# blasif/cocons

Hardware: NVIDIA B200
Metric: neg2loglik evals/sec (assembly+Cholesky) at n=50k (higher is better)
Workload: dtype f64

## Files before the change

### cocons_b200/csrc/capi.cu

```cuda
#include <algorithm>
#include <atomic>
#include <iterator>
#include <cmath>
#include <cstdarg>
#include <cstdio>
#include <cstring>
#include <mutex>
#include <vector>

#include "../../include/cocons_b200.h"
#include "common.cuh"

namespace cocons {

static thread_local char g_err[512] = "";
void set_error(const char* fmt, ...) {
  va_list ap;
  va_start(ap, fmt);
  vsnprintf(g_err, sizeof(g_err), fmt, ap);
  va_end(ap);
}

static std::atomic<long long> g_launches{0};
void note_launch(int count) { g_launches += count; }
// ... 1534 lines not shown
    cudaSetDevice(c->device);
    morton_order(n, locs, c->perm.data());
    c->hX.assign(X, X + (size_t)n * p);
    c->rank_x = -1;
    cudaFree(c->dInv), cudaFree(c->dTapCol), cudaFree(c->dTapRow), cudaFree(c->dTap);
    c->dInv = c->dTapCol = c->dTapRow = nullptr, c->dTap = nullptr, c->tap_nnz = 0;
    std::vector<int> orig((size_t)c->n_pad);
    for (int64_t s = 0; s < c->n_pad; ++s) orig[(size_t)s] = (s < n) ? (int)c->perm[(size_t)s] : (int)s;
    COCONS_CUDA_TRY(cudaMemcpy(c->dOrig, orig.data(), sizeof(int) * c->n_pad, cudaMemcpyHostToDevice));
    if ((rc = upload_sorted(c, X, p, c->dX)) || (rc = upload_sorted(c, locs, 2, c->dLocs)) ||
        (rc = upload_sorted(c, z, r, c->dZ)))
      return rc;
  }
  if (kind == COCONS_PROFILE) {
    if (!xb || q <= 0) {
      set_error("neg2loglik_dense: COCONS_PROFILE needs x_betas");
      return COCONS_ERR_ARG;
    }
    if ((rc = cocons_ctx_set_xbetas(g_ws, q, xb))) return rc;
  }
  return cocons_n2ll(g_ws, kind, theta6, limits, mean_p, logdet, quad, logdet_w, rank_x);
}


__global__ void fill_kernel(double* p, int64_t count, double scale) {
  const int64_t i = (int64_t)blockIdx.x * blockDim.x + threadIdx.x;
  if (i < count) p[i] = scale * (double)(((uint64_t)i * 2654435761ull) % 1024ull) / 1024.0;
}

int cocons_bench_syrk(int device, int64_t n, int64_t k, int reps, double* ms_per_rep) {
  int rc = check_device(device);
  if (rc) return rc;
  if (n % kTile || k % 16 || !ms_per_rep || reps <= 0) {
    set_error("bench_syrk: n must be a multiple of 128 and k of 16");
    return COCONS_ERR_ARG;
  }
  double *dC = nullptr, *dP = nullptr;
  COCONS_CUDA_TRY(cudaMalloc(&dC, sizeof(double) * n * n));
  if (cudaMalloc(&dP, sizeof(double) * n * k) != cudaSuccess) {
    cudaFree(dC);
    set_error("bench_syrk: out of device memory");
    return COCONS_ERR_ALLOC;
  }
  fill_kernel<<<(unsigned)((n * n + 255) / 256), 256>>>(dC, n * n, 1.0);
  fill_kernel<<<(unsigned)((n * k + 255) / 256), 256>>>(dP, n * k, 1e-3);
  cudaEvent_t e0, e1;
  cudaEventCreate(&e0), cudaEventCreate(&e1);
  launch_gemm_nt(0, n, n, k, dP, n, dP, n, dC, n, 1, nullptr);
  cudaEventRecord(e0);
  for (int i = 0; i < reps; ++i) launch_gemm_nt(0, n, n, k, dP, n, dP, n, dC, n, 1, nullptr);
  cudaEventRecord(e1);
  cudaError_t e = cudaEventSynchronize(e1);
  float ms = 0;
  cudaEventElapsedTime(&ms, e0, e1);
  cudaEventDestroy(e0), cudaEventDestroy(e1);
  cudaFree(dC), cudaFree(dP);
  if (e != cudaSuccess) {
    set_error("bench_syrk: %s", cudaGetErrorString(e));
    return COCONS_ERR_CUDA;
  }
  *ms_per_rep = ms / reps;
  return 0;
}

int cocons_trailing_update(int device, int64_t m, const double* P, double* C, int path, int reps, double* ms_per_rep) {
  int rc = check_device(device);
  if (rc) return rc;
  if (m <= 0 || m % kTile || (path != 0 && path != 1) || reps < 0 || (reps > 0 && !ms_per_rep) || (!P != !C)) {
    set_error("trailing_update: m must be a positive multiple of 128, path 0 or 1, and P and C both given or both "
              "null");
    return COCONS_ERR_ARG;
  }
  if (path == 1 && !g_syrk_i8.update) {
    set_error("trailing_update: this build of the library has no split-int8 update");
    return COCONS_ERR_STATE;
  }
  const int64_t k = kSyrkI8K;
  double *dC = nullptr, *dP = nullptr, *dS = nullptr;
  int8_t* dQ = nullptr;
  int* dInfo = nullptr;
  if (cudaMalloc(&dC, sizeof(double) * m * m) != cudaSuccess || cudaMalloc(&dP, sizeof(double) * m * k) != cudaSuccess ||
      (path == 1 && (cudaMalloc(&dQ, (size_t)kSyrkI8BytesPerRow * m) != cudaSuccess ||
                     cudaMalloc(&dS, sizeof(double) * m) != cudaSuccess ||
                     cudaMalloc(&dInfo, sizeof(int)) != cudaSuccess))) {
    cudaFree(dC), cudaFree(dP), cudaFree(dQ), cudaFree(dS), cudaFree(dInfo);
    set_error("trailing_update: out of device memory");
    return COCONS_ERR_ALLOC;
  }
  if (dInfo) cudaMemsetAsync(dInfo, 0, sizeof(int), nullptr);
  if (P) {
    cudaMemcpy(dP, P, sizeof(double) * m * k, cudaMemcpyHostToDevice);
    cudaMemcpy(dC, C, sizeof(double) * m * m, cudaMemcpyHostToDevice);
  } else {
    cudaMemsetAsync(dC, 0x3F, sizeof(double) * m * m, nullptr);
    cudaMemsetAsync(dP, 0x3F, sizeof(double) * m * k, nullptr);
  }
  auto run = [&]() {
    if (path == 1) {
      g_syrk_i8.split(dP, m, m, dQ, dS, nullptr);
      g_syrk_i8.update(m, m, dQ, dS, 0, 0, dC, m, 1, dInfo, nullptr);
    } else {
      launch_gemm_nt(0, m, m, k, dP, m, dP, m, dC, m, 1, nullptr);
    }
  };
  run();
  if (C) cudaMemcpy(C, dC, sizeof(double) * m * m, cudaMemcpyDeviceToHost);
  cudaEvent_t e0, e1;
  cudaEventCreate(&e0), cudaEventCreate(&e1);
  cudaEventRecord(e0);
  for (int i = 0; i < reps; ++i) run();
  cudaEventRecord(e1);
  cudaError_t e = cudaEventSynchronize(e1);
  float ms = 0;
  cudaEventElapsedTime(&ms, e0, e1);
  cudaEventDestroy(e0), cudaEventDestroy(e1);
  int info = 0;
  if (dInfo && e == cudaSuccess) e = cudaMemcpy(&info, dInfo, sizeof(int), cudaMemcpyDeviceToHost);
  cudaFree(dC), cudaFree(dP), cudaFree(dQ), cudaFree(dS), cudaFree(dInfo);
  if (e != cudaSuccess) {
    set_error("trailing_update: %s", cudaGetErrorString(e));
    return COCONS_ERR_CUDA;
  }
  if (info != 0) {
    set_error("trailing_update: a barrier wait of the split-int8 update gave up");
    return COCONS_ERR_CUDA;
  }
  if (reps > 0) *ms_per_rep = ms / reps;
  return 0;
}

}
```

### cocons_b200/csrc/chol.cu

```cuda
#include <algorithm>
#include <type_traits>

#include "../../include/cocons_b200.h"
#include "common.cuh"
#include "tile_order.cuh"

namespace cocons {

#ifndef COCONS_GEMM_RELEASE
#define COCONS_GEMM_RELEASE 1
#endif
constexpr int GBM = 128, GBK = 16, GSTAGES = 4;
constexpr int GLDA = GBM + 4;
constexpr int kGemmMapped = 2;

template <int BN, int NU = 2>
struct GemmCfg {
  static constexpr int kWarpI = 16 * NU;
  static constexpr int kWarpsI = GBM / kWarpI;
  static constexpr int kWarpsJ = BN / 32;
  static constexpr int kThreads = kWarpsI * kWarpsJ * 32;
  static constexpr int kLdb = BN + 4;
  static constexpr int kStageDoubles = GBK * (GLDA + kLdb);
  static constexpr int kSmemBytes = GSTAGES * kStageDoubles * (int)sizeof(double);
// ... 544 lines not shown
    if (s >= 0) {
      PROBEB(2 + 3 * s);
      if (fail) return;
      double* Dt = Tb + pblk(s, s);
      int t = 0;
      for (int a = s + 1; a < PNB; ++a, ++t)
        if ((t & 7) == warp) bmm16<0>(Lb + pblk(a, s), Lb + pblk(a, s), 1, PBS, Dt, PBS, 1, lane);
      for (int c = 0; c < s; ++c, ++t)
        if ((t & 7) == warp) bmm16<0>(Tb + pblk(s, c), Dt, 1, PBS, Tb + pblk(s, c), 1, PBS, lane);
      __syncthreads();
      PROBEB(3 + 3 * s);
    }
    if (warp == 0) {
      if (s + 1 < PNB) {
        if (s >= 0) {
          bmm16<1>(Lb + pblk(s + 1, s + 1), Lb + pblk(s + 1, s), 1, PBS, Lb + pblk(s + 1, s), PBS, 1, lane);
          __syncwarp();
        }
        potrf_diag_block(Lb + pblk(s + 1, s + 1), Tb + pblk(s + 1, s + 1), rinvs, lane, &fail, info,
                         first_index + (s + 1) * PB);
      }
    } else if (s >= 0) {
      int t = 0;
      for (int a = s + 1; a < PNB; ++a) {
        for (int b = s + 1; b <= a; ++b) {
          if (a == s + 1 && b == s + 1) continue;
          if (t++ % 7 == warp - 1)
            bmm16<1>(Lb + pblk(a, b), Lb + pblk(a, s), 1, PBS, Lb + pblk(b, s), PBS, 1, lane);
        }
        for (int c = 0; c <= s; ++c)
          if (t++ % 7 == warp - 1)
            bmm16<1>(Tb + pblk(a, c), Lb + pblk(a, s), 1, PBS, Tb + pblk(s, c), 1, PBS, lane);
      }
    }
    __syncthreads();
    if (s >= 0) PROBEB(4 + 3 * s);
  }

#pragma unroll 4
  for (int idx = tid; idx < PT * PT / 2; idx += 256) {
    const int i = (2 * idx) & (PT - 1), j = (2 * idx) >> 7;
    const int a = i >> 4, b = j >> 4;
    double2 l, w;
    l.x = l.y = w.x = w.y = 0.0;
    if (a >= b) {
      const int off = pblk(a, b) + (j & 15) * PBS + (i & 15);
      const double2 lv = *reinterpret_cast<const double2*>(Lb + off);
      const double2 wv = *reinterpret_cast<const double2*>(Tb + off);
      if (i >= j) l.x = lv.x, w.x = wv.x;
      if (i + 1 >= j) l.y = lv.y, w.y = wv.y;
    }
    *reinterpret_cast<double2*>(A + (int64_t)j * ld + i) = l;
    *reinterpret_cast<double2*>(Winv + j * PT + i) = w;
  }
  PROBEB(30);
}

void launch_potrf_tile(double* A, int64_t ld, double* Winv, int* info, int first_index, cudaStream_t st) {
  static int variant = -1;
  static bool attr_done[16] = {};
  if (variant < 0) {
    const char* e = getenv("COCONS_POTRF");
    variant = e ? atoi(e) : 2;
  }
  note_launch();
  if (variant == 1) {
    potrf_tile_kernel<<<1, 256, 0, st>>>(A, ld, Winv, info, first_index);
    return;
  }
  int dev = 0;
  cudaGetDevice(&dev);
  if (dev < 16 && !attr_done[dev]) {
    cudaFuncSetAttribute(potrf_tile_blocked_kernel, cudaFuncAttributeMaxDynamicSharedMemorySize, kPotrfBlockedSmem);
    attr_done[dev] = true;
  }
  potrf_tile_blocked_kernel<<<1, 256, kPotrfBlockedSmem, st>>>(A, ld, Winv, info, first_index);
}

SyrkI8Ops g_syrk_i8 = {nullptr, nullptr};

int chol_workspace_create(int64_t n_pad, CholWorkspace* ws, bool with_i8) {
  ws->winv = nullptr, ws->info = nullptr, ws->panel_stream = nullptr, ws->ev_a = nullptr, ws->ev_p = nullptr;
  ws->ev_k0 = nullptr, ws->ev_k1 = nullptr;
  ws->i8_slices = nullptr, ws->i8_scale = nullptr;
  int lo = 0, hi = 0;
  cudaDeviceGetStreamPriorityRange(&lo, &hi);
  if (const char* e = getenv("COCONS_PANEL_PRIORITY"))
    if (atoi(e) == 0) hi = 0;
  if (cudaMalloc(&ws->winv, sizeof(double) * (n_pad / kTile) * kTile * kTile) != cudaSuccess ||
      cudaMalloc(&ws->info, sizeof(int)) != cudaSuccess ||
      cudaStreamCreateWithPriority(&ws->panel_stream, cudaStreamNonBlocking, hi) != cudaSuccess ||
      cudaEventCreateWithFlags(&ws->ev_a, cudaEventDisableTiming) != cudaSuccess ||
      cudaEventCreateWithFlags(&ws->ev_p, cudaEventDisableTiming) != cudaSuccess ||
      cudaEventCreate(&ws->ev_k0) != cudaSuccess || cudaEventCreate(&ws->ev_k1) != cudaSuccess) {
    chol_workspace_destroy(ws);
    return COCONS_ERR_ALLOC;
  }
  if (with_i8 && g_syrk_i8.update && n_pad >= kSyrkI8MinPad &&
      (cudaMalloc(&ws->i8_slices, (size_t)kSyrkI8BytesPerRow * n_pad) != cudaSuccess ||
       cudaMalloc(&ws->i8_scale, sizeof(double) * n_pad) != cudaSuccess)) {
    chol_workspace_destroy(ws);
    return COCONS_ERR_ALLOC;
  }
  return 0;
}

void chol_workspace_destroy(CholWorkspace* ws) {
  cudaFree(ws->winv), cudaFree(ws->info);
  if (ws->i8_slices) cudaFree(ws->i8_slices);
  if (ws->i8_scale) cudaFree(ws->i8_scale);
  ws->i8_slices = nullptr, ws->i8_scale = nullptr;
  if (ws->panel_stream) cudaStreamDestroy(ws->panel_stream);
  if (ws->ev_a) cudaEventDestroy(ws->ev_a);
  if (ws->ev_p) cudaEventDestroy(ws->ev_p);
  if (ws->ev_k0) cudaEventDestroy(ws->ev_k0);
  if (ws->ev_k1) cudaEventDestroy(ws->ev_k1);
  ws->ev_k0 = nullptr, ws->ev_k1 = nullptr;
  ws->winv = nullptr, ws->info = nullptr, ws->panel_stream = nullptr, ws->ev_a = nullptr, ws->ev_p = nullptr;
}

void factor_panel(double* A, int64_t n_pad, int64_t ld, const CholWorkspace& ws, int64_t J0, int64_t jb,
                  cudaStream_t st) {
  for (int64_t jj = J0; jj < J0 + jb; ++jj) {
    double* Ajj = A + jj * kTile * ld + jj * kTile;
    double* Wjj = ws.winv + jj * (int64_t)kTile * kTile;
    launch_potrf_tile(Ajj, ld, Wjj, ws.info, (int)(jj * kTile), st);
    const int64_t below = n_pad - (jj + 1) * kTile;
    if (below <= 0) continue;
    double* panel = Ajj + kTile;
    launch_gemm_nt(1, below, kTile, kTile, panel, ld, Wjj, kTile, panel, ld, 0, st);
    const int64_t rest = (J0 + jb - jj - 1) * kTile;
    if (rest > 0) launch_gemm_nt(0, below, rest, kTile, panel, ld, panel, ld, Ajj + kTile * ld + kTile, ld, 1, st);
  }
}

int chol_outer(int64_t n_pad) {
  static int forced = -1;
  if (forced < 0) {
    const char* e = getenv("COCONS_CHOL_OUTER");
    forced = e ? std::max(1, std::min(atoi(e), 16)) : 0;
  }
  if (forced > 0) return forced;
  return n_pad >= 16384 ? 6 : (n_pad >= 8192 ? 4 : 2);
}

constexpr int64_t kSyrkI8MinRows = 16384;

static bool syrk_i8_enabled(const CholWorkspace& ws) {
  if (!g_syrk_i8.update || !ws.i8_slices) return false;
  const char* e = getenv("COCONS_SYRK_I8");
  return !(e && atoi(e) == 0);
}

int chol_factor(double* A, int64_t n_pad, int64_t ld, CholWorkspace ws, cudaStream_t st) {
  cudaMemsetAsync(ws.info, 0, sizeof(int), st);
  const bool i8 = syrk_i8_enabled(ws);
  const int64_t nt = n_pad / kTile;
  const int64_t outer = chol_outer(n_pad);
  static int lookahead = -1;
  if (lookahead < 0) {
    const char* e = getenv("COCONS_CHOL_LOOKAHEAD");
    lookahead = e ? atoi(e) : 1;
  }
  cudaStream_t ps = lookahead ? ws.panel_stream : st;
  factor_panel(A, n_pad, ld, ws, 0, std::min<int64_t>(outer, nt), st);
  for (int64_t J0 = 0; J0 < nt; J0 += outer) {
    const int64_t jb = std::min<int64_t>(outer, nt - J0);
    const int64_t done = (J0 + jb) * kTile;
    const int64_t trail = n_pad - done;
    if (trail <= 0) break;
    const int64_t nb_next = std::min<int64_t>(outer, nt - (J0 + jb));
    const int64_t wnext = nb_next * kTile;
    const double* P = A + J0 * kTile * ld + done;
    const int64_t rest = trail - wnext;
    const bool split = i8 && jb * kTile == kSyrkI8K && trail >= kSyrkI8MinRows;
    if (split) {
      g_syrk_i8.split(P, ld, trail, ws.i8_slices, ws.i8_scale, st);
      g_syrk_i8.update(trail, wnext, ws.i8_slices, ws.i8_scale, 0, 0, A + done * ld + done, ld, 1, ws.info, st);
    } else {
      launch_gemm_nt(0, trail, wnext, jb * kTile, P, ld, P, ld, A + done * ld + done, ld, 1, st);
    }
    cudaEventRecord(ws.ev_a, st);
    cudaStreamWaitEvent(ps, ws.ev_a, 0);
    factor_panel(A, n_pad, ld, ws, J0 + jb, nb_next, ps);
    cudaEventRecord(ws.ev_p, ps);
    if (rest > 0) {
      double* C2 = A + (done + wnext) * ld + done + wnext;
      if (J0 == 0) cudaEventRecord(ws.ev_k0, st);
      if (split) {
        if (J0 == 0) g_syrk_i8.split(P + wnext, ld, rest, ws.i8_slices + wnext * kSyrkI8BytesPerRow,
                                     ws.i8_scale + wnext, st);
        g_syrk_i8.update(rest, rest, ws.i8_slices, ws.i8_scale, wnext, wnext, C2, ld, 1, ws.info, st);
      } else {
        const double* P2 = P + wnext;
        launch_gemm_nt(0, rest, rest, jb * kTile, P2, ld, P2, ld, C2, ld, 1, st);
      }
      if (J0 == 0) cudaEventRecord(ws.ev_k1, st);
    }
    cudaStreamWaitEvent(st, ws.ev_p, 0);
  }
  return 0;
}

}
```

### cocons_b200/csrc/common.cuh

```cuda
#ifndef COCONS_COMMON_CUH
#define COCONS_COMMON_CUH

#include <cuda_runtime.h>
#include <stdint.h>

namespace cocons {

constexpr int kTile = 128;

enum SiteField {
  SF_X = 0,
  SF_Y,
  SF_R,
  SF_A2,
  SF_RA,
  SF_CS,
  SF_P22,
  SF_E22,
  SF_P12,
  SF_E12,
  SF_NU,
  SF_SIG,
  SF_W,
  SF_AMP,
// ... 1 lines not shown
  SF_COUNT
};

struct SiteTable {
  double* base;
  int64_t stride;
  const int* orig;
  __host__ __device__ const double* f(int k) const { return base + (int64_t)k * stride; }
  __host__ __device__ double* fw(int k) const { return base + (int64_t)k * stride; }
};

enum SmoothMode {
  SM_GENERAL = 0,
  SM_HALF = 1,
  SM_THREEHALF = 2,
  SM_FIVEHALF = 3,
  SM_CLASSIC = 4,
  SM_DEGENERATE = 5
};

void set_error(const char* fmt, ...);
void note_launch(int count = 1);

#define COCONS_CUDA_TRY(expr)                                                                  \
  do {                                                                                         \
    cudaError_t _e = (expr);                                                                   \
    if (_e != cudaSuccess) {                                                                   \
      ::cocons::set_error("%s failed at %s:%d: %s", #expr, __FILE__, __LINE__, cudaGetErrorString(_e)); \
      return COCONS_ERR_CUDA;                                                                  \
    }                                                                                          \
  } while (0)

int smooth_mode_for(int par, int p, const double* theta6_host, const double* limits_host, double* nu_fixed);
void launch_site_stage(int64_t n, int64_t n_fill, int p, const double* dX, int64_t ldx, const double* dlocs,
                       int64_t ldl, const double* dtheta6, double lim0, double lim1, int mode, SiteTable T,
                       cudaStream_t st);
void launch_assemble_lower(int64_t n, int64_t n_out, SiteTable T, double global_range, double nu_fixed, int mode,
                           double* C, int64_t ld, cudaStream_t st);
void launch_assemble_panel(int64_t n, int64_t n_out, SiteTable T, double global_range, double nu_fixed, int mode,
                           double* slab, int64_t ld, int col_tile0, int ncol_tiles, cudaStream_t st);
void launch_assemble_cyclic(int64_t n, int64_t n_out, SiteTable T, double global_range, double nu_fixed, int mode,
                            double* slab, int64_t ld, int world, int rank, int64_t nlocal, cudaStream_t st);
void launch_assemble_cross(int64_t m, int64_t n, SiteTable Tpred, SiteTable Ttrain, double global_range, double* C,
                           int64_t ld, cudaStream_t st);
void launch_symmetrize(int64_t n, double* C, int64_t ld, cudaStream_t st);
void morton_order(int64_t n, const double* locs, int64_t* perm);

enum TaperField { TF_X = 0, TF_Y, TF_R, TF_SIG, TF_NU, TF_DV, TF_COUNT };
struct TaperTable {
  double* base;
  int64_t stride;
  __host__ __device__ const double* f(int k) const { return base + (int64_t)k * stride; }
  __host__ __device__ double* fw(int k) const { return base + (int64_t)k * stride; }
};
void launch_taper_site_stage(int64_t n, int p, const double* dX, int64_t ldx, const double* dlocs, int64_t ldl,
                             const double* dtheta6, double lim0, double lim1, int mode, int pred_rows, TaperTable T,
                             cudaStream_t st);
enum TaperSinkKind { TS_VECTOR = 0, TS_LOWER = 1, TS_ROWS = 2, TS_TILED = 3 };
struct TaperSink {
  int kind;
  double* out;
  const double* taper;
  const int* inv;
  double* A;
  int64_t ld;
  int64_t row0;
  const int64_t* tiles;
};
constexpr int kTaperTiled = 8;
void launch_taper_entries(int64_t e0, int64_t count, int64_t nrows, const int* dcol, const int* drow, TaperTable R,
                          TaperTable C, int square, int mode, double nu_fixed, TaperSink S, cudaStream_t st);
void launch_taper_pad_diag(int64_t n, int64_t n_pad, double* A, int64_t ld, cudaStream_t st);

struct CholWorkspace {
  double* winv;
  int* info;
  cudaStream_t panel_stream;
  cudaEvent_t ev_a, ev_p;
  cudaEvent_t ev_k0, ev_k1;
  unsigned* solve_ctrl;
  int* solve_units;
  double* solve_part;
  int solve_nunits, solve_nchunks;
  int8_t* i8_slices;
  double* i8_scale;
};
constexpr int kSolveMaxRhs = 8;
constexpr int kSolveChunk = 16;
int chol_workspace_create(int64_t n_pad, CholWorkspace* ws, bool with_i8 = false);
void chol_workspace_destroy(CholWorkspace* ws);
void factor_panel(double* A, int64_t n_pad, int64_t ld, const CholWorkspace& ws, int64_t J0, int64_t jb,
                  cudaStream_t st);
int chol_factor(double* A, int64_t n_pad, int64_t ld, CholWorkspace ws, cudaStream_t st);
int chol_outer(int64_t n_pad);
void launch_potrf_tile(double* A, int64_t ld, double* Winv, int* info, int first_index, cudaStream_t st);
void launch_gemm_nt(int mode, int64_t M, int64_t N, int64_t K, const double* A, int64_t lda, const double* B,
                    int64_t ldb, double* C, int64_t ldc, int lower_only, cudaStream_t st);

constexpr int kSyrkI8K = 768;
constexpr int64_t kSyrkI8MinPad = 16384;
constexpr int64_t kSyrkI8BytesPerRow = 8 * kSyrkI8K;
struct SyrkI8Ops {
  void (*split)(const double* P, int64_t ld, int64_t m, int8_t* q, double* scale, cudaStream_t st);
  void (*update)(int64_t M, int64_t N, const int8_t* q, const double* scale, int64_t a_row0, int64_t b_row0,
                 double* C, int64_t ldc, int lower_only, int* info, cudaStream_t st);
};
extern SyrkI8Ops g_syrk_i8;

void launch_logdet(const double* L, int64_t n, int64_t ld, double* out, cudaStream_t st);
void forward_solve(const double* L, int64_t n_pad, int64_t ld, const double* winv, double* B, int64_t ldb, int nrhs,
                   cudaStream_t st);
int solve_workspace_create(int64_t n_pad, CholWorkspace* ws);
}
#include <vector>
namespace cocons {
int build_solve_units(int64_t T, std::vector<int>* out);
void solve_workspace_destroy(CholWorkspace* ws);
void forward_solve_ws(const double* L, int64_t n_pad, int64_t ld, const CholWorkspace& ws, double* B, int64_t ldb,
                      int nrhs, cudaStream_t st);
void launch_gram(const double* Y, int64_t n, int64_t ldy, int k, double* G, cudaStream_t st);

}

#endif
```

### cocons_b200/csrc/syrk_i8.cu

```cuda
#include "../../include/cocons_b200.h"
#include "common.cuh"
#include "tile_order.cuh"

namespace cocons {
namespace {

constexpr int kSlices = 8;
constexpr int kWeights = kSlices;
constexpr int kHiTop = 5;
constexpr int kChunk = 32;
constexpr int kChunks = kSyrkI8K / kChunk;
constexpr int kRowsA = 128, kRowsB = 64;
constexpr uint32_t kSliceBytesA = kRowsA * kChunk;
constexpr uint32_t kSliceBytesB = kRowsB * kChunk;
constexpr uint32_t kBlockBytes = kSlices * kSliceBytesA;
constexpr uint32_t kStageBytes = kSlices * (kSliceBytesA + kSliceBytesB);
constexpr int kStages = 4;
constexpr int kEpiWarps = 8;
constexpr int kThreads = 32 * (2 + kEpiWarps);
constexpr int kSplitThreads = 128;
constexpr int kSmemBytes = kStages * kStageBytes + 1024;
constexpr int kTmemCols = 512;
static_assert(kWeights * kRowsB <= kTmemCols, "the accumulators must fit tensor memory");

__device__ __forceinline__ uint32_t smem_u32(const void* p) { return (uint32_t)__cvta_generic_to_shared(p); }
__device__ __forceinline__ void mbar_init(uint32_t bar, uint32_t count) {
  asm volatile("mbarrier.init.shared::cta.b64 [%0], %1;" ::"r"(bar), "r"(count));
}
__device__ __forceinline__ void mbar_expect_tx(uint32_t bar, uint32_t bytes) {
  asm volatile("mbarrier.arrive.expect_tx.shared::cta.b64 _, [%0], %1;" ::"r"(bar), "r"(bytes) : "memory");
}
__device__ __forceinline__ void mbar_arrive(uint32_t bar) {
  asm volatile("mbarrier.arrive.shared::cta.b64 _, [%0];" ::"r"(bar) : "memory");
}
__device__ __forceinline__ bool mbar_try(uint32_t bar, uint32_t parity) {
  uint32_t ok;
  asm volatile(
      "{\n"
      ".reg .pred p;\n"
      "mbarrier.try_wait.parity.shared::cta.b64 p, [%1], %2;\n"
      "selp.u32 %0, 1, 0, p;\n"
      "}"
      : "=r"(ok)
      : "r"(bar), "r"(parity)
      : "memory");
  return ok != 0;
}
__device__ __forceinline__ uint64_t globaltimer_ns() {
  uint64_t t;
  asm volatile("mov.u64 %0, %%globaltimer;" : "=l"(t));
  return t;
}
constexpr uint64_t kWaitLimitNs = 2000000000ull;
__device__ __noinline__ bool mbar_wait(uint32_t bar, uint32_t parity, int* info) {
  if (mbar_try(bar, parity)) return true;
  const uint64_t t0 = globaltimer_ns();
  while (!mbar_try(bar, parity))
    if (globaltimer_ns() - t0 > kWaitLimitNs) {
      atomicCAS(info, 0, COCONS_ERR_CUDA);
      return false;
    }
  return true;
}
__device__ __forceinline__ void bulk_g2s(uint32_t dst, const void* src, uint32_t bytes, uint32_t bar) {
  asm volatile("cp.async.bulk.shared::cluster.global.mbarrier::complete_tx::bytes [%0], [%1], %2, [%3];" ::"r"(dst),
               "l"(src), "r"(bytes), "r"(bar)
               : "memory");
}
__device__ __forceinline__ void bulk_g2s_mc(uint32_t dst, const void* src, uint32_t bytes, uint32_t bar, uint16_t mask) {
  asm volatile(
      "cp.async.bulk.shared::cluster.global.mbarrier::complete_tx::bytes.multicast::cluster [%0], [%1], %2, [%3], "
      "%4;" ::"r"(dst),
      "l"(src), "r"(bytes), "r"(bar), "h"(mask)
      : "memory");
}

__device__ __forceinline__ uint64_t sw32_desc(uint32_t saddr) {
  return (uint64_t)((saddr & 0x3FFFF) >> 4) | (1ull << 16) | ((uint64_t)(256 >> 4) << 32) | (1ull << 46) |
         (6ull << 61);
}
__host__ __device__ constexpr uint32_t idesc_i8(int nblk) {
  return (2u << 4) | (1u << 7) | (1u << 10) | ((uint32_t)(nblk * kRowsB >> 3) << 17) | ((uint32_t)(kRowsA >> 4) << 24);
}

__device__ __forceinline__ void umma_i8(uint32_t dtmem, uint64_t adesc, uint64_t bdesc, uint32_t idesc, uint32_t acc) {
  asm volatile(
      "{\n"
      ".reg .pred p;\n"
      "setp.ne.b32 p, %4, 0;\n"
      "tcgen05.mma.cta_group::1.kind::i8 [%0], %1, %2, %3, p;\n"
      "}" ::"r"(dtmem),
      "l"(adesc), "l"(bdesc), "r"(idesc), "r"(acc));
}

struct SlicePairs {
  int t, u0, nblk;
};
constexpr int kMmas = 12;
__host__ __device__ constexpr SlicePairs slice_pairs(int k) {
  constexpr SlicePairs p[kMmas] = {{1, 1, 4}, {1, 5, 4}, {2, 1, 4}, {3, 1, 4}, {4, 1, 4}, {5, 1, 4},
                                   {6, 1, 3}, {7, 1, 2}, {8, 1, 1}, {2, 5, 3}, {3, 5, 2}, {4, 5, 1}};
  return p[k];
}
__device__ __forceinline__ void umma_commit(uint32_t bar) {
  asm volatile("tcgen05.commit.cta_group::1.mbarrier::arrive::one.shared::cluster.b64 [%0];" ::"r"(bar) : "memory");
}
__device__ __forceinline__ void umma_commit_mc(uint32_t bar, uint16_t mask) {
  asm volatile(
      "tcgen05.commit.cta_group::1.mbarrier::arrive::one.shared::cluster.multicast::cluster.b64 [%0], %1;" ::"r"(bar),
      "h"(mask)
      : "memory");
}

#define TMEM_LD8(taddr, r)                                                                                      \
  asm volatile("tcgen05.ld.sync.aligned.32x32b.x8.b32 {%0,%1,%2,%3,%4,%5,%6,%7}, [%8];"                          \
               : "=r"(r[0]), "=r"(r[1]), "=r"(r[2]), "=r"(r[3]), "=r"(r[4]), "=r"(r[5]), "=r"(r[6]), "=r"(r[7]) \
               : "r"(taddr))

__device__ __forceinline__ void cluster_sync() {
  asm volatile("barrier.cluster.arrive.release.aligned;\nbarrier.cluster.wait.acquire.aligned;" ::: "memory");
}

__host__ __device__ __forceinline__ uint32_t sw32_offset(int i, int b) {
  const uint32_t off = (uint32_t)i * kChunk + (uint32_t)b;
  return off ^ (((off >> 7) & 1u) << 4);
}

}

__global__ void __launch_bounds__(kSplitThreads) syrk_i8_split_kernel(const double* __restrict__ P, int64_t ld,
                                                                  int8_t* __restrict__ q, double* __restrict__ scale) {
  const int i = threadIdx.x;
  const int64_t tile = blockIdx.x, row = tile * kRowsA + i;
  const double* p = P + row;
  double m = 0.0;
  for (int k = 0; k < kSyrkI8K; ++k) m = fmax(m, fabs(p[(int64_t)k * ld]));
  int e = 0;
  if (m > 0.0) {
    frexp(m, &e);
    if (ldexp(m, 7 - e) >= 127.5) ++e;
  }
  scale[row] = ldexp(1.0, e);
  const double inv = ldexp(1.0, -e);
  int8_t* qt = q + tile * kChunks * (int64_t)kBlockBytes;
  for (int c = 0; c < kChunks; ++c) {
#pragma unroll
    for (int h = 0; h < 2; ++h) {
      uint32_t w[kSlices][4];
#pragma unroll
      for (int k4 = 0; k4 < 4; ++k4) {
#pragma unroll
        for (int t = 0; t < kSlices; ++t) w[t][k4] = 0;
#pragma unroll
        for (int kb = 0; kb < 4; ++kb) {
          double x = p[(int64_t)(c * kChunk + 16 * h + 4 * k4 + kb) * ld] * inv;
#pragma unroll
          for (int t = 0; t < kSlices; ++t) {
            const double y = x * 128.0;
            const double a = rint(y);
            x = y - a;
            w[t][k4] |= ((uint32_t)(int)a & 0xFFu) << (8 * kb);
          }
        }
      }
#pragma unroll
      for (int t = 0; t < kSlices; ++t)
        *reinterpret_cast<uint4*>(qt + (int64_t)c * kBlockBytes + t * kSliceBytesA + sw32_offset(i, 16 * h)) =
            make_uint4(w[t][0], w[t][1], w[t][2], w[t][3]);
    }
  }
}

namespace {

#ifndef COCONS_I8_CLUSTER_M
#define COCONS_I8_CLUSTER_M 1
#endif
#ifndef COCONS_I8_CLUSTER_N
#define COCONS_I8_CLUSTER_N 2
#endif
constexpr int kCM = COCONS_I8_CLUSTER_M, kCN = COCONS_I8_CLUSTER_N, kCtas = kCM * kCN;
static_assert((kCM == 1 || kCM == 2) && (kCN == 1 || kCN == 2), "clusters of 1 or 2 tile rows and columns");
constexpr int kW = 2 * kCM / kCN, kBand = kBandRows / kCM;

#ifdef COCONS_I8_PROBE
__device__ unsigned long long g_i8_probe[8];
#define I8_PROBE(...) __VA_ARGS__
#else
#define I8_PROBE(...)
#endif

__device__ __forceinline__ void super_tile(int64_t st, int ni, int nj, int lower_only, int rm, int cn, int& bi, int& bj,
                                           bool& store) {
  int R, Cc;
  tile_decode<kW, kBand>(st, (ni + kCM - 1) / kCM, nj / kCN, lower_only, R, Cc);
  bi = R * kCM + rm, bj = Cc * kCN + cn;
  store = bi < ni && (!lower_only || bi >= bj / 2);
}

}

__global__ void __launch_bounds__(kThreads, 1)
    syrk_i8_update_kernel(int ni, int nj, int lower_only, const int8_t* __restrict__ qa, const double* __restrict__ sa,
                          const int8_t* __restrict__ qb, const double* __restrict__ sb, double* C, int64_t ldc,
                          int* info) {
  extern __shared__ uint8_t smem_raw[];
  __shared__ __align__(8) uint64_t bars[2 * kStages + 2];
  __shared__ uint32_t tmem_slot;
  I8_PROBE(const long long t_start = clock64();)
  const int tid = threadIdx.x, warp = tid >> 5, lane = tid & 31;
  const int rank = (int)(blockIdx.x % kCtas), rm = rank / kCN, cn = rank % kCN;
  const int64_t cluster = blockIdx.x / kCtas, nclusters = gridDim.x / kCtas;
  const int64_t nsuper = total_tiles<kW, kBand>((ni + kCM - 1) / kCM, nj / kCN, lower_only);
  const uint32_t stage0 = (smem_u32(smem_raw) + 1023u) & ~1023u;
  const uint32_t full0 = smem_u32(bars), empty0 = full0 + 8 * kStages;
  const uint32_t tmem_full = full0 + 16 * kStages, tmem_empty = tmem_full + 8;
  if (tid == 0) {
    for (int s = 0; s < kStages; ++s) {
      mbar_init(full0 + 8 * s, 1);
      mbar_init(empty0 + 8 * s, kCtas);
    }
    mbar_init(tmem_full, 1);
    mbar_init(tmem_empty, 32 * kEpiWarps);
    asm volatile("fence.mbarrier_init.release.cluster;" ::: "memory");
  }
  if (warp == 0) {
    asm volatile("tcgen05.alloc.cta_group::1.sync.aligned.shared::cta.b32 [%0], %1;" ::"r"(smem_u32(&tmem_slot)),
                 "r"(kTmemCols));
    asm volatile("tcgen05.relinquish_alloc_permit.cta_group::1.sync.aligned;");
  }
  asm volatile("tcgen05.fence::before_thread_sync;" ::: "memory");
  __syncthreads();
  asm volatile("tcgen05.fence::after_thread_sync;" ::: "memory");
  if (kCtas > 1) cluster_sync();
  const uint32_t tmem = tmem_slot;
  I8_PROBE(unsigned long long p_first = 0, p_full = 0, p_empty = 0, p_epi = 0, p_tmem = 0, p_tiles = 0;)

  if (warp == 0) {
    if (lane == 0) {
      constexpr uint16_t all = (uint16_t)((1u << kCtas) - 1);
      uint16_t row_mask = 0, col_mask = 0;
      for (int r = 0; r < kCtas; ++r) {
        if (r / kCN == rm) row_mask |= (uint16_t)(1u << r);
        if (r % kCN == cn) col_mask |= (uint16_t)(1u << r);
      }
      (void)all;
      uint32_t it = 0;
      bool ok = true;
      for (int64_t st = cluster; ok && st < nsuper; st += nclusters) {
        int bi, bj;
        bool store;
        super_tile(st, ni, nj, lower_only, rm, cn, bi, bj, store);
        const int8_t* a = qa + (int64_t)(bi < ni ? bi : ni - 1) * kChunks * kBlockBytes + cn * (kBlockBytes / kCN);
        const int8_t* b = qb + (int64_t)(bj >> 1) * kChunks * kBlockBytes + (bj & 1) * kSliceBytesB;
        for (int c = 0; c < kChunks; ++c, ++it) {
          const uint32_t slot = it % kStages;
          if (it >= kStages) {
            I8_PROBE(const long long t0 = clock64();)
            if (!mbar_wait(empty0 + 8 * slot, ((it / kStages) - 1) & 1, info)) {
              ok = false;
              break;
            }
            I8_PROBE(p_empty += clock64() - t0;)
          }
          const uint32_t fb = full0 + 8 * slot, da = stage0 + slot * kStageBytes, db = da + kSlices * kSliceBytesA;
          mbar_expect_tx(fb, kStageBytes);
          const uint32_t aoff = cn * (kBlockBytes / kCN);
          if (kCN > 1)
            bulk_g2s_mc(da + aoff, a + (int64_t)c * kBlockBytes, kBlockBytes / kCN, fb, row_mask);
          else
            bulk_g2s(da + aoff, a + (int64_t)c * kBlockBytes, kBlockBytes / kCN, fb);
#pragma unroll
          for (int t = rm; t < kSlices; t += kCM) {
            if (kCM > 1)
              bulk_g2s_mc(db + t * kSliceBytesB, b + (int64_t)c * kBlockBytes + t * kSliceBytesA, kSliceBytesB, fb,
                          col_mask);
            else
              bulk_g2s(db + t * kSliceBytesB, b + (int64_t)c * kBlockBytes + t * kSliceBytesA, kSliceBytesB, fb);
          }
        }
      }
      for (uint32_t e = 0; ok && e < kStages; ++e, ++it)
        if (it >= kStages) ok = mbar_wait(empty0 + 8 * (it % kStages), ((it / kStages) - 1) & 1, info);
    }
  } else if (warp == 1) {
    if (lane == 0) {
      constexpr uint16_t all = (uint16_t)((1u << kCtas) - 1);
      uint32_t it = 0, tl = 0;
      bool ok = true;
      for (int64_t st = cluster; ok && st < nsuper; st += nclusters, ++tl) {
        if (tl > 0) {
          I8_PROBE(const long long t0 = clock64();)
          if (!mbar_wait(tmem_empty, (tl - 1) & 1, info)) break;
          I8_PROBE(p_tmem += clock64() - t0;)
          asm volatile("tcgen05.fence::after_thread_sync;" ::: "memory");
        }
        for (int c = 0; c < kChunks; ++c, ++it) {
          const uint32_t slot = it % kStages;
          I8_PROBE(const long long t0 = clock64();)
          if (!mbar_wait(full0 + 8 * slot, (it / kStages) & 1, info)) {
            ok = false;
            break;
          }
          I8_PROBE(const long long t1 = clock64(); p_full += t1 - t0; if (it == 0) p_first = t1 - t_start;)
          asm volatile("tcgen05.fence::after_thread_sync;" ::: "memory");
          const uint32_t da = stage0 + slot * kStageBytes, db = da + kSlices * kSliceBytesA;
#pragma unroll
          for (int k = 0; k < kMmas; ++k) {
            const SlicePairs q = slice_pairs(k);
            umma_i8(tmem + (uint32_t)(q.t + q.u0 - 2) * kRowsB, sw32_desc(da + (q.t - 1) * kSliceBytesA),
                    sw32_desc(db + (q.u0 - 1) * kSliceBytesB), idesc_i8(q.nblk), (c > 0 || k >= 2) ? 1u : 0u);
          }
          if (kCtas > 1)
            umma_commit_mc(empty0 + 8 * slot, all);
          else
            umma_commit(empty0 + 8 * slot);
        }
        if (ok) umma_commit(tmem_full);
        I8_PROBE(++p_tiles;)
      }
    }
  } else {
    const int quarter = warp & 3, h = (warp - 2) >> 2, r = 32 * quarter + lane;
    const uint32_t trow = tmem + ((uint32_t)(32 * quarter) << 16) + (uint32_t)(32 * h);
    uint32_t tl = 0;
    for (int64_t st = cluster; st < nsuper; st += nclusters, ++tl) {
      int bi, bj;
      bool store;
      super_tile(st, ni, nj, lower_only, rm, cn, bi, bj, store);
      double* Cg = C + (int64_t)(bj * kRowsB + 32 * h) * ldc + (int64_t)bi * kRowsA + r;
      if (store)
#pragma unroll 4
        for (int j = 0; j < 32; ++j) asm volatile("prefetch.global.L2 [%0];" ::"l"(Cg + (int64_t)j * ldc));
      if (!mbar_wait(tmem_full, tl & 1, info)) break;
      I8_PROBE(const long long t0 = clock64();)
      asm volatile("tcgen05.fence::after_thread_sync;" ::: "memory");
      double v[32];
#pragma unroll
      for (int j0 = 0; j0 < 32; j0 += 8) {
        uint32_t acc[kWeights][8];
#pragma unroll
        for (int w = 0; w < kWeights; ++w) TMEM_LD8(trow + (uint32_t)(w * kRowsB + j0), acc[w]);
        asm volatile("tcgen05.wait::ld.sync.aligned;" ::: "memory");
#pragma unroll
        for (int jj = 0; jj < 8; ++jj) {
          int64_t hi = 0, lo = 0;
#pragma unroll
          for (int w = 0; w < kWeights; ++w) {
            const int64_t s = (int64_t)(int32_t)acc[w][jj];
            if (w + 2 <= kHiTop)
              hi = hi * 128 + s;
            else
              lo = lo * 128 + s;
          }
          v[j0 + jj] = (double)hi * 0x1p-35 + (double)lo * 0x1p-63;
        }
      }
      asm volatile("tcgen05.fence::before_thread_sync;" ::: "memory");
      mbar_arrive(tmem_empty);
      if (store) {
        const double si = sa[(int64_t)bi * kRowsA + r];
        const double* sbj = sb + (int64_t)bj * kRowsB + 32 * h;
#pragma unroll
        for (int j = 0; j < 32; ++j) {
          double* p = Cg + (int64_t)j * ldc;
          __stcs(p, __ldcs(p) - (v[j] * si) * sbj[j]);
        }
      }
      I8_PROBE(if (tid == 64) p_epi += clock64() - t0;)
    }
  }
  __syncwarp();
  asm volatile("tcgen05.fence::before_thread_sync;" ::: "memory");
  __syncthreads();
  if (kCtas > 1) cluster_sync();
  if (warp == 0) {
    asm volatile("tcgen05.fence::after_thread_sync;" ::: "memory");
    asm volatile("tcgen05.dealloc.cta_group::1.sync.aligned.b32 %0, %1;" ::"r"(tmem), "r"(kTmemCols));
  }
  I8_PROBE(if (tid == 32) {
    atomicAdd(&g_i8_probe[0], p_first), atomicAdd(&g_i8_probe[1], p_full), atomicAdd(&g_i8_probe[4], p_tmem);
    atomicAdd(&g_i8_probe[5], (unsigned long long)(clock64() - t_start)), atomicAdd(&g_i8_probe[6], p_tiles);
    atomicAdd(&g_i8_probe[7], 1ull);
  } if (tid == 0) atomicAdd(&g_i8_probe[2], p_empty);
           if (tid == 64) atomicAdd(&g_i8_probe[3], p_epi);)
}

namespace {

static_assert(kHiTop == 5 && kSlices == 8, "the epilogue's 2^-35 and 2^-63 are for 8 slices with weights 2..5 high");

void split(const double* P, int64_t ld, int64_t m, int8_t* q, double* scale, cudaStream_t st) {
  if (m <= 0) return;
  note_launch();
  syrk_i8_split_kernel<<<(unsigned)(m / kRowsA), kSplitThreads, 0, st>>>(P, ld, q, scale);
}

void update(int64_t M, int64_t N, const int8_t* q, const double* scale, int64_t a_row0, int64_t b_row0, double* C,
            int64_t ldc, int lower_only, int* info, cudaStream_t st) {
  if (M <= 0 || N <= 0) return;
  cudaLaunchConfig_t cfg = {};
  cudaLaunchAttribute attr[1];
  attr[0].id = cudaLaunchAttributeClusterDimension;
  attr[0].val.clusterDim.x = kCtas, attr[0].val.clusterDim.y = 1, attr[0].val.clusterDim.z = 1;
  cfg.blockDim = dim3(kThreads);
  cfg.dynamicSmemBytes = kSmemBytes;
  cfg.stream = st;
  cfg.attrs = attr;
  cfg.numAttrs = 1;
  static int max_clusters[16] = {};
  int dev = 0;
  cudaGetDevice(&dev);
  int clusters = dev < 16 ? max_clusters[dev] : 0;
  if (clusters <= 0) {
    cudaFuncSetAttribute(syrk_i8_update_kernel, cudaFuncAttributeMaxDynamicSharedMemorySize, kSmemBytes);
    cfg.gridDim = dim3(kCtas);
    if (cudaOccupancyMaxActiveClusters(&clusters, syrk_i8_update_kernel, &cfg) != cudaSuccess || clusters <= 0) {
      int sms = 0;
      cudaDeviceGetAttribute(&sms, cudaDevAttrMultiProcessorCount, dev);
      clusters = sms / kCtas > 0 ? sms / kCtas : 1;
    }
    if (dev < 16) max_clusters[dev] = clusters;
  }
  const int ni = (int)(M / kRowsA), nj = (int)(N / kRowsB);
  const int64_t nsuper = total_tiles<kW, kBand>((ni + kCM - 1) / kCM, nj / kCN, lower_only);
  cfg.gridDim = dim3((unsigned)(kCtas * (nsuper < clusters ? nsuper : clusters)));
  const int8_t* qa = q + a_row0 / kRowsA * kChunks * (int64_t)kBlockBytes;
  const int8_t* qb = q + b_row0 / kRowsA * kChunks * (int64_t)kBlockBytes;
  note_launch();
  cudaLaunchKernelEx(&cfg, syrk_i8_update_kernel, ni, nj, lower_only, qa, scale + a_row0, qb, scale + b_row0, C, ldc,
                     info);
}

struct Register {
  Register() { g_syrk_i8 = SyrkI8Ops{split, update}; }
} register_syrk_i8;

}
}

#ifdef COCONS_I8_PROBE
extern "C" int cocons_i8_probe_read(unsigned long long* out) {
  if (cudaMemcpyFromSymbol(out, cocons::g_i8_probe, sizeof(cocons::g_i8_probe)) != cudaSuccess) return -1;
  const unsigned long long zero[8] = {};
  return cudaMemcpyToSymbol(cocons::g_i8_probe, zero, sizeof(zero)) == cudaSuccess ? 0 : -1;
}
#endif
```

Before: 1.501.

## Share int8 trailing update across streams via dynamic tile tickets and double-buffered splits

The int8 SYRK update kernel now pulls its super-tiles from a global atomic ticket instead of a static cluster stride. Rank 0 of each cluster publishes each ticket to the other CTAs through cluster-shared mbarriers. Chol_factor uses this to launch a second, small update on the panel stream with a reserved SM budget, working on the same trailing block concurrently with the main-stream launch; the main launch gives up those SMs. It also pre-splits the next panel into a second int8 buffer on the lookahead stream. The aim is to keep SMs busy while the panel factorization runs, at the cost of per-tile atomics, cluster barrier traffic, extra memsets and double the slice memory.

```diff
diff --git a/cocons_b200/csrc/capi.cu b/cocons_b200/csrc/capi.cu
--- a/cocons_b200/csrc/capi.cu
+++ b/cocons_b200/csrc/capi.cu
@@ -1640,7 +1640,7 @@
   if (cudaMalloc(&dC, sizeof(double) * m * m) != cudaSuccess || cudaMalloc(&dP, sizeof(double) * m * k) != cudaSuccess ||
       (path == 1 && (cudaMalloc(&dQ, (size_t)kSyrkI8BytesPerRow * m) != cudaSuccess ||
                      cudaMalloc(&dS, sizeof(double) * m) != cudaSuccess ||
-                     cudaMalloc(&dInfo, sizeof(int)) != cudaSuccess))) {
+                     cudaMalloc(&dInfo, 2 * sizeof(int)) != cudaSuccess))) {
     cudaFree(dC), cudaFree(dP), cudaFree(dQ), cudaFree(dS), cudaFree(dInfo);
     set_error("trailing_update: out of device memory");
     return COCONS_ERR_ALLOC;
@@ -1655,8 +1655,10 @@
   }
   auto run = [&]() {
     if (path == 1) {
+      unsigned* ticket = reinterpret_cast<unsigned*>(dInfo + 1);
       g_syrk_i8.split(dP, m, m, dQ, dS, nullptr);
-      g_syrk_i8.update(m, m, dQ, dS, 0, 0, dC, m, 1, dInfo, nullptr);
+      cudaMemsetAsync(ticket, 0, sizeof(unsigned), nullptr);
+      g_syrk_i8.update(m, m, dQ, dS, 0, 0, dC, m, 1, ticket, 0, dInfo, nullptr);
     } else {
       launch_gemm_nt(0, m, m, k, dP, m, dP, m, dC, m, 1, nullptr);
     }
diff --git a/cocons_b200/csrc/chol.cu b/cocons_b200/csrc/chol.cu
--- a/cocons_b200/csrc/chol.cu
+++ b/cocons_b200/csrc/chol.cu
@@ -650,7 +650,8 @@
 int chol_workspace_create(int64_t n_pad, CholWorkspace* ws, bool with_i8) {
   ws->winv = nullptr, ws->info = nullptr, ws->panel_stream = nullptr, ws->ev_a = nullptr, ws->ev_p = nullptr;
   ws->ev_k0 = nullptr, ws->ev_k1 = nullptr;
-  ws->i8_slices = nullptr, ws->i8_scale = nullptr;
+  ws->i8_slices[0] = ws->i8_slices[1] = nullptr, ws->i8_scale[0] = ws->i8_scale[1] = nullptr;
+  ws->i8_tickets = nullptr;
   int lo = 0, hi = 0;
   cudaDeviceGetStreamPriorityRange(&lo, &hi);
   if (const char* e = getenv("COCONS_PANEL_PRIORITY"))
@@ -664,20 +665,30 @@
     chol_workspace_destroy(ws);
     return COCONS_ERR_ALLOC;
   }
-  if (with_i8 && g_syrk_i8.update && n_pad >= kSyrkI8MinPad &&
-      (cudaMalloc(&ws->i8_slices, (size_t)kSyrkI8BytesPerRow * n_pad) != cudaSuccess ||
-       cudaMalloc(&ws->i8_scale, sizeof(double) * n_pad) != cudaSuccess)) {
-    chol_workspace_destroy(ws);
-    return COCONS_ERR_ALLOC;
+  if (with_i8 && g_syrk_i8.update && n_pad >= kSyrkI8MinPad) {
+    for (int b = 0; b < 2; ++b)
+      if (cudaMalloc(&ws->i8_slices[b], (size_t)kSyrkI8BytesPerRow * n_pad) != cudaSuccess ||
+          cudaMalloc(&ws->i8_scale[b], sizeof(double) * n_pad) != cudaSuccess) {
+        chol_workspace_destroy(ws);
+        return COCONS_ERR_ALLOC;
+      }
+    if (cudaMalloc(&ws->i8_tickets, 2 * sizeof(unsigned)) != cudaSuccess) {
+      chol_workspace_destroy(ws);
+      return COCONS_ERR_ALLOC;
+    }
   }
   return 0;
 }
 
 void chol_workspace_destroy(CholWorkspace* ws) {
   cudaFree(ws->winv), cudaFree(ws->info);
-  if (ws->i8_slices) cudaFree(ws->i8_slices);
-  if (ws->i8_scale) cudaFree(ws->i8_scale);
-  ws->i8_slices = nullptr, ws->i8_scale = nullptr;
+  for (int b = 0; b < 2; ++b) {
+    if (ws->i8_slices[b]) cudaFree(ws->i8_slices[b]);
+    if (ws->i8_scale[b]) cudaFree(ws->i8_scale[b]);
+    ws->i8_slices[b] = nullptr, ws->i8_scale[b] = nullptr;
+  }
+  if (ws->i8_tickets) cudaFree(ws->i8_tickets);
+  ws->i8_tickets = nullptr;
   if (ws->panel_stream) cudaStreamDestroy(ws->panel_stream);
   if (ws->ev_a) cudaEventDestroy(ws->ev_a);
   if (ws->ev_p) cudaEventDestroy(ws->ev_p);
@@ -715,9 +726,19 @@
 constexpr int64_t kSyrkI8MinRows = 16384;
 
 static bool syrk_i8_enabled(const CholWorkspace& ws) {
-  if (!g_syrk_i8.update || !ws.i8_slices) return false;
+  if (!g_syrk_i8.update || !ws.i8_slices[1] || !ws.i8_tickets) return false;
   const char* e = getenv("COCONS_SYRK_I8");
   return !(e && atoi(e) == 0);
+}
+
+static int chain_sms(int64_t m) {
+#ifdef COCONS_CHOL_RESERVE_SMS
+  (void)m;
+  return COCONS_CHOL_RESERVE_SMS;
+#else
+  const int64_t r = (12 * 49152 + m - 1) / m;
+  return (int)std::min<int64_t>(48, std::max<int64_t>(8, (r + 1) & ~int64_t(1)));
+#endif
 }
 
 int chol_factor(double* A, int64_t n_pad, int64_t ld, CholWorkspace ws, cudaStream_t st) {
@@ -731,7 +752,17 @@
     lookahead = e ? atoi(e) : 1;
   }
   cudaStream_t ps = lookahead ? ws.panel_stream : st;
+  auto int8_panel = [&](int64_t J0) {
+    const int64_t jb = std::min<int64_t>(outer, nt - J0);
+    return i8 && jb * kTile == kSyrkI8K && n_pad - (J0 + jb) * kTile >= kSyrkI8MinRows;
+  };
+  auto split_panel = [&](int64_t J0, int b, cudaStream_t s) {
+    const int64_t done = (J0 + std::min<int64_t>(outer, nt - J0)) * kTile;
+    g_syrk_i8.split(A + J0 * kTile * ld + done, ld, n_pad - done, ws.i8_slices[b], ws.i8_scale[b], s);
+  };
   factor_panel(A, n_pad, ld, ws, 0, std::min<int64_t>(outer, nt), st);
+  int buf = 0;
+  bool presplit = false;
   for (int64_t J0 = 0; J0 < nt; J0 += outer) {
     const int64_t jb = std::min<int64_t>(outer, nt - J0);
     const int64_t done = (J0 + jb) * kTile;
@@ -741,24 +772,31 @@
     const int64_t wnext = nb_next * kTile;
     const double* P = A + J0 * kTile * ld + done;
     const int64_t rest = trail - wnext;
-    const bool split = i8 && jb * kTile == kSyrkI8K && trail >= kSyrkI8MinRows;
+    const bool split = int8_panel(J0);
+    int8_t* q = split ? ws.i8_slices[buf] : nullptr;
+    double* sc = split ? ws.i8_scale[buf] : nullptr;
     if (split) {
-      g_syrk_i8.split(P, ld, trail, ws.i8_slices, ws.i8_scale, st);
-      g_syrk_i8.update(trail, wnext, ws.i8_slices, ws.i8_scale, 0, 0, A + done * ld + done, ld, 1, ws.info, st);
+      if (!presplit) split_panel(J0, buf, st);
+      cudaMemsetAsync(ws.i8_tickets, 0, 2 * sizeof(unsigned), st);
+      g_syrk_i8.update(trail, wnext, q, sc, 0, 0, A + done * ld + done, ld, 1, ws.i8_tickets, 0, ws.info, st);
     } else {
       launch_gemm_nt(0, trail, wnext, jb * kTile, P, ld, P, ld, A + done * ld + done, ld, 1, st);
     }
     cudaEventRecord(ws.ev_a, st);
     cudaStreamWaitEvent(ps, ws.ev_a, 0);
     factor_panel(A, n_pad, ld, ws, J0 + jb, nb_next, ps);
+    presplit = lookahead && int8_panel(J0 + jb);
+    if (presplit) split_panel(J0 + jb, buf ^ 1, ps);
+    double* C2 = A + (done + wnext) * ld + done + wnext;
+    const bool cont = lookahead && split && J0 > 0 && rest > 0;
+    const int reserve = cont ? chain_sms(rest) : 0;
+    if (cont) g_syrk_i8.update(rest, rest, q, sc, wnext, wnext, C2, ld, 1, ws.i8_tickets + 1, reserve, ws.info, ps);
     cudaEventRecord(ws.ev_p, ps);
     if (rest > 0) {
-      double* C2 = A + (done + wnext) * ld + done + wnext;
       if (J0 == 0) cudaEventRecord(ws.ev_k0, st);
       if (split) {
-        if (J0 == 0) g_syrk_i8.split(P + wnext, ld, rest, ws.i8_slices + wnext * kSyrkI8BytesPerRow,
-                                     ws.i8_scale + wnext, st);
-        g_syrk_i8.update(rest, rest, ws.i8_slices, ws.i8_scale, wnext, wnext, C2, ld, 1, ws.info, st);
+        if (J0 == 0) g_syrk_i8.split(P + wnext, ld, rest, q + wnext * kSyrkI8BytesPerRow, sc + wnext, st);
+        g_syrk_i8.update(rest, rest, q, sc, wnext, wnext, C2, ld, 1, ws.i8_tickets + 1, -reserve, ws.info, st);
       } else {
         const double* P2 = P + wnext;
         launch_gemm_nt(0, rest, rest, jb * kTile, P2, ld, P2, ld, C2, ld, 1, st);
@@ -766,6 +804,7 @@
       if (J0 == 0) cudaEventRecord(ws.ev_k1, st);
     }
     cudaStreamWaitEvent(st, ws.ev_p, 0);
+    if (presplit) buf ^= 1;
   }
   return 0;
 }
diff --git a/cocons_b200/csrc/common.cuh b/cocons_b200/csrc/common.cuh
--- a/cocons_b200/csrc/common.cuh
+++ b/cocons_b200/csrc/common.cuh
@@ -107,8 +107,9 @@
   int* solve_units;
   double* solve_part;
   int solve_nunits, solve_nchunks;
-  int8_t* i8_slices;
-  double* i8_scale;
+  int8_t* i8_slices[2];
+  double* i8_scale[2];
+  unsigned* i8_tickets;
 };
 constexpr int kSolveMaxRhs = 8;
 constexpr int kSolveChunk = 16;
@@ -128,7 +129,7 @@
 struct SyrkI8Ops {
   void (*split)(const double* P, int64_t ld, int64_t m, int8_t* q, double* scale, cudaStream_t st);
   void (*update)(int64_t M, int64_t N, const int8_t* q, const double* scale, int64_t a_row0, int64_t b_row0,
-                 double* C, int64_t ldc, int lower_only, int* info, cudaStream_t st);
+                 double* C, int64_t ldc, int lower_only, unsigned* ticket, int ctas, int* info, cudaStream_t st);
 };
 extern SyrkI8Ops g_syrk_i8;
 
diff --git a/cocons_b200/csrc/syrk_i8.cu b/cocons_b200/csrc/syrk_i8.cu
--- a/cocons_b200/csrc/syrk_i8.cu
+++ b/cocons_b200/csrc/syrk_i8.cu
@@ -21,6 +21,8 @@
 constexpr int kSplitThreads = 128;
 constexpr int kSmemBytes = kStages * kStageBytes + 1024;
 constexpr int kTmemCols = 512;
+constexpr int kSched = 4;
+constexpr uint32_t kSchedReaders = 2 + kEpiWarps;
 static_assert(kWeights * kRowsB <= kTmemCols, "the accumulators must fit tensor memory");
 
 __device__ __forceinline__ uint32_t smem_u32(const void* p) { return (uint32_t)__cvta_generic_to_shared(p); }
@@ -33,17 +35,29 @@
 __device__ __forceinline__ void mbar_arrive(uint32_t bar) {
   asm volatile("mbarrier.arrive.shared::cta.b64 _, [%0];" ::"r"(bar) : "memory");
 }
+template <bool kCluster>
 __device__ __forceinline__ bool mbar_try(uint32_t bar, uint32_t parity) {
   uint32_t ok;
-  asm volatile(
-      "{\n"
-      ".reg .pred p;\n"
-      "mbarrier.try_wait.parity.shared::cta.b64 p, [%1], %2;\n"
-      "selp.u32 %0, 1, 0, p;\n"
-      "}"
-      : "=r"(ok)
-      : "r"(bar), "r"(parity)
-      : "memory");
+  if (kCluster)
+    asm volatile(
+        "{\n"
+        ".reg .pred p;\n"
+        "mbarrier.try_wait.parity.acquire.cluster.shared::cta.b64 p, [%1], %2;\n"
+        "selp.u32 %0, 1, 0, p;\n"
+        "}"
+        : "=r"(ok)
+        : "r"(bar), "r"(parity)
+        : "memory");
+  else
+    asm volatile(
+        "{\n"
+        ".reg .pred p;\n"
+        "mbarrier.try_wait.parity.shared::cta.b64 p, [%1], %2;\n"
+        "selp.u32 %0, 1, 0, p;\n"
+        "}"
+        : "=r"(ok)
+        : "r"(bar), "r"(parity)
+        : "memory");
   return ok != 0;
 }
 __device__ __forceinline__ uint64_t globaltimer_ns() {
@@ -52,10 +66,11 @@
   return t;
 }
 constexpr uint64_t kWaitLimitNs = 2000000000ull;
+template <bool kCluster = false>
 __device__ __noinline__ bool mbar_wait(uint32_t bar, uint32_t parity, int* info) {
-  if (mbar_try(bar, parity)) return true;
+  if (mbar_try<kCluster>(bar, parity)) return true;
   const uint64_t t0 = globaltimer_ns();
-  while (!mbar_try(bar, parity))
+  while (!mbar_try<kCluster>(bar, parity))
     if (globaltimer_ns() - t0 > kWaitLimitNs) {
       atomicCAS(info, 0, COCONS_ERR_CUDA);
       return false;
@@ -116,6 +131,18 @@
   asm volatile("tcgen05.ld.sync.aligned.32x32b.x8.b32 {%0,%1,%2,%3,%4,%5,%6,%7}, [%8];"                          \
                : "=r"(r[0]), "=r"(r[1]), "=r"(r[2]), "=r"(r[3]), "=r"(r[4]), "=r"(r[5]), "=r"(r[6]), "=r"(r[7]) \
                : "r"(taddr))
+
+__device__ __forceinline__ uint32_t mapa(uint32_t saddr, uint32_t rank) {
+  uint32_t r;
+  asm volatile("mapa.shared::cluster.u32 %0, %1, %2;" : "=r"(r) : "r"(saddr), "r"(rank));
+  return r;
+}
+__device__ __forceinline__ void st_cluster_u32(uint32_t caddr, uint32_t v) {
+  asm volatile("st.shared::cluster.u32 [%0], %1;" ::"r"(caddr), "r"(v) : "memory");
+}
+__device__ __forceinline__ void mbar_arrive_cluster(uint32_t caddr) {
+  asm volatile("mbarrier.arrive.release.cluster.shared::cluster.b64 _, [%0];" ::"r"(caddr) : "memory");
+}
 
 __device__ __forceinline__ void cluster_sync() {
   asm volatile("barrier.cluster.arrive.release.aligned;\nbarrier.cluster.wait.acquire.aligned;" ::: "memory");
@@ -203,19 +230,24 @@
 __global__ void __launch_bounds__(kThreads, 1)
     syrk_i8_update_kernel(int ni, int nj, int lower_only, const int8_t* __restrict__ qa, const double* __restrict__ sa,
                           const int8_t* __restrict__ qb, const double* __restrict__ sb, double* C, int64_t ldc,
-                          int* info) {
+                          unsigned* ticket, int* info) {
   extern __shared__ uint8_t smem_raw[];
-  __shared__ __align__(8) uint64_t bars[2 * kStages + 2];
+  __shared__ __align__(8) uint64_t bars[2 * kStages + 2 + 2 * kSched];
   __shared__ uint32_t tmem_slot;
+  __shared__ uint32_t sched_tile[kSched];
   I8_PROBE(const long long t_start = clock64();)
   const int tid = threadIdx.x, warp = tid >> 5, lane = tid & 31;
   const int rank = (int)(blockIdx.x % kCtas), rm = rank / kCN, cn = rank % kCN;
-  const int64_t cluster = blockIdx.x / kCtas, nclusters = gridDim.x / kCtas;
   const int64_t nsuper = total_tiles<kW, kBand>((ni + kCM - 1) / kCM, nj / kCN, lower_only);
   const uint32_t stage0 = (smem_u32(smem_raw) + 1023u) & ~1023u;
   const uint32_t full0 = smem_u32(bars), empty0 = full0 + 8 * kStages;
   const uint32_t tmem_full = full0 + 16 * kStages, tmem_empty = tmem_full + 8;
+  const uint32_t sched_full = tmem_empty + 8, sched_empty = sched_full + 8 * kSched;
   if (tid == 0) {
+    for (int s = 0; s < kSched; ++s) {
+      mbar_init(sched_full + 8 * s, 1);
+      mbar_init(sched_empty + 8 * s, kCtas * kSchedReaders);
+    }
     for (int s = 0; s < kStages; ++s) {
       mbar_init(full0 + 8 * s, 1);
       mbar_init(empty0 + 8 * s, kCtas);
@@ -235,6 +267,22 @@
   if (kCtas > 1) cluster_sync();
   const uint32_t tmem = tmem_slot;
   I8_PROBE(unsigned long long p_first = 0, p_full = 0, p_empty = 0, p_epi = 0, p_tmem = 0, p_tiles = 0;)
+  auto publish = [&](uint32_t k) -> bool {
+    const uint32_t s = k % kSched;
+    if (k >= kSched && !mbar_wait<true>(sched_empty + 8 * s, ((k / kSched) - 1) & 1, info)) return false;
+    const uint32_t t = atomicAdd(ticket, 1u);
+    for (int r = 0; r < kCtas; ++r) {
+      st_cluster_u32(mapa(smem_u32(&sched_tile[s]), (uint32_t)r), t);
+      mbar_arrive_cluster(mapa(sched_full + 8 * s, (uint32_t)r));
+    }
+    return true;
+  };
+  auto take = [&](uint32_t k) -> int64_t {
+    const uint32_t s = k % kSched;
+    if (!mbar_wait<true>(sched_full + 8 * s, (k / kSched) & 1, info)) return -1;
+    return (int64_t)*reinterpret_cast<volatile uint32_t*>(&sched_tile[s]);
+  };
+  auto release = [&](uint32_t k) { mbar_arrive_cluster(mapa(sched_empty + 8 * (k % kSched), 0)); };
 
   if (warp == 0) {
     if (lane == 0) {
@@ -246,8 +294,12 @@
       }
       (void)all;
       uint32_t it = 0;
-      bool ok = true;
-      for (int64_t st = cluster; ok && st < nsuper; st += nclusters) {
+      bool ok = rank != 0 || publish(0);
+      for (uint32_t k = 0; ok; ++k) {
+        const int64_t st = take(k);
+        release(k);
+        if (st < 0 || st >= nsuper) break;
+        if (rank == 0 && !publish(k + 1)) break;
         int bi, bj;
         bool store;
         super_tile(st, ni, nj, lower_only, rm, cn, bi, bj, store);
@@ -288,7 +340,10 @@
       constexpr uint16_t all = (uint16_t)((1u << kCtas) - 1);
       uint32_t it = 0, tl = 0;
       bool ok = true;
-      for (int64_t st = cluster; ok && st < nsuper; st += nclusters, ++tl) {
+      for (; ok; ++tl) {
+        const int64_t st = take(tl);
+        release(tl);
+        if (st < 0 || st >= nsuper) break;
         if (tl > 0) {
           I8_PROBE(const long long t0 = clock64();)
           if (!mbar_wait(tmem_empty, (tl - 1) & 1, info)) break;
@@ -323,8 +378,11 @@
   } else {
     const int quarter = warp & 3, h = (warp - 2) >> 2, r = 32 * quarter + lane;
     const uint32_t trow = tmem + ((uint32_t)(32 * quarter) << 16) + (uint32_t)(32 * h);
-    uint32_t tl = 0;
-    for (int64_t st = cluster; st < nsuper; st += nclusters, ++tl) {
+    for (uint32_t tl = 0;; ++tl) {
+      const int64_t st = take(tl);
+      __syncwarp();
+      if (lane == 0) release(tl);
+      if (st < 0 || st >= nsuper) break;
       int bi, bj;
       bool store;
       super_tile(st, ni, nj, lower_only, rm, cn, bi, bj, store);
@@ -397,7 +455,7 @@
 }
 
 void update(int64_t M, int64_t N, const int8_t* q, const double* scale, int64_t a_row0, int64_t b_row0, double* C,
-            int64_t ldc, int lower_only, int* info, cudaStream_t st) {
+            int64_t ldc, int lower_only, unsigned* ticket, int ctas, int* info, cudaStream_t st) {
   if (M <= 0 || N <= 0) return;
   cudaLaunchConfig_t cfg = {};
   cudaLaunchAttribute attr[1];
@@ -424,12 +482,17 @@
   }
   const int ni = (int)(M / kRowsA), nj = (int)(N / kRowsB);
   const int64_t nsuper = total_tiles<kW, kBand>((ni + kCM - 1) / kCM, nj / kCN, lower_only);
+  if (ctas <= 0)
+    clusters -= (-ctas + kCtas - 1) / kCtas;
+  else if (ctas / kCtas < clusters)
+    clusters = ctas / kCtas;
+  if (clusters < 1) clusters = 1;
   cfg.gridDim = dim3((unsigned)(kCtas * (nsuper < clusters ? nsuper : clusters)));
   const int8_t* qa = q + a_row0 / kRowsA * kChunks * (int64_t)kBlockBytes;
   const int8_t* qb = q + b_row0 / kRowsA * kChunks * (int64_t)kBlockBytes;
   note_launch();
   cudaLaunchKernelEx(&cfg, syrk_i8_update_kernel, ni, nj, lower_only, qa, scale + a_row0, qb, scale + b_row0, C, ldc,
-                     info);
+                     ticket, info);
 }
 
 struct Register {
```

Result: faster. 1.521 (median of 6 runs) (+1.3%).
